# rik1599/SimplexOnCuda

Measured on AMD Instinct MI355X. Metric: simplex pivots/sec + HBM GB/s on gaussian update, dense m×n tableau, higher is better.
Workload: dtype f64

## Files before the change

simplexoncuda_amd/csrc/sx_kernels.hip:

```cpp

#include <float.h>

#include "sx_argmin.hpp"
#include "sx_common.hpp"

namespace {

__global__ __launch_bounds__(512) void k_argmin_pass1(const double *__restrict__ v, int L, TilePart *out,
                                                      const DevState *st) {
    if (st != nullptr && st->status != SX_NOT_ENDED) return;
    __shared__ double s_v[16];
    __shared__ int s_i[16];
    double mv = DBL_MAX;
    int mi = -1;
    for (int i = blockIdx.x * SX_TILE + threadIdx.x; i < L; i += SX_TILE * gridDim.x) {
        const double c = v[i];
        if (cmp_eps(c, mv) < 0) {
            mv = c;
            mi = i;
        }
    }
    block_argmin512(mv, mi, s_v, s_i);
    if (threadIdx.x == 0) {
        out[blockIdx.x].v = mv;
// ... 437 lines not shown
    double v = DBL_MAX;
    int i = -1;
    if ((int)threadIdx.x < B1) {
        double cv;
        int ci, ce;
        load_tile_sc1(enter_parts + threadIdx.x, cv, ci, ce);
        if (cmp_eps(cv, v) < 0) {
            v = cv;
            i = ci;
        }
    }
    half_argmin(v, i);
    __syncthreads();
    if (lane == 0) {
        s_v[h] = v;
        s_i[h] = i;
    }
    __syncthreads();
    if (threadIdx.x < 32) {
        v = (threadIdx.x < 8) ? s_v[threadIdx.x] : DBL_MAX;
        i = (threadIdx.x < 8) ? s_i[threadIdx.x] : -1;
        half_argmin(v, i);
        if (threadIdx.x == 0) {
            st->e_next = i;
            st->dmin_next = v;
            st->ticket_d = 0;
        }
    }
}

typedef unsigned long long u64;

__device__ __forceinline__ void drain() { asm volatile("s_waitcnt vmcnt(0)" ::: "memory"); }

#define SX_PAYBITS 11
#define SX_PAYMASK ((1u << SX_PAYBITS) - 1u)
#define SX_NOIDX 0x3FFu
__device__ __forceinline__ unsigned make_tag(unsigned B, int q) {
    return ((B & 0x7FFFu) << (6 + SX_PAYBITS)) | ((unsigned)q << SX_PAYBITS);
}

__device__ __forceinline__ void put_g(u64 *g, unsigned data, unsigned tag) {
    __hip_atomic_store(g, ((u64)tag << 32) | data, __ATOMIC_RELAXED, __HIP_MEMORY_SCOPE_AGENT);
}
__device__ __forceinline__ double gd(unsigned lo, unsigned hi) {
    return __longlong_as_double((long long)(((u64)hi << 32) | lo));
}
__device__ __forceinline__ u64 ld_sc1(const u64 *p) {
    return __hip_atomic_load(const_cast<u64 *>(p), __ATOMIC_RELAXED, __HIP_MEMORY_SCOPE_AGENT);
}
__device__ __forceinline__ unsigned ld_sc1(const unsigned *p) {
    return __hip_atomic_load(const_cast<unsigned *>(p), __ATOMIC_RELAXED, __HIP_MEMORY_SCOPE_AGENT);
}

#define SX_GB4 4
#define SX_GBS 16
#define SX_OBJ_TILES 160

__device__ __forceinline__ void st_sc1(double *p, double v) {
    __hip_atomic_store(reinterpret_cast<u64 *>(p), (u64)__double_as_longlong(v), __ATOMIC_RELAXED,
                       __HIP_MEMORY_SCOPE_AGENT);
}
__device__ __forceinline__ double ld_sc1d(const double *p) {
    return __longlong_as_double((long long)ld_sc1(reinterpret_cast<const u64 *>(p)));
}
struct IdOff {
    __device__ __forceinline__ int operator()(int k) const { return k; }
};
struct Rec4Val {
    __device__ __forceinline__ int operator()(int k) const { return (k >> 1) * SX_GBS + (k & 1); }
};
struct Rec4AllFrom {
    int k0;
    __device__ __forceinline__ int operator()(int k) const { return ((k0 + k) >> 2) * SX_GBS + ((k0 + k) & 3); }
};
struct Rec4All {
    __device__ __forceinline__ int operator()(int k) const { return (k >> 2) * SX_GBS + (k & 3); }
};

__device__ __forceinline__ u64 ld_sys(const u64 *p) {
    return __hip_atomic_load(const_cast<u64 *>(p), __ATOMIC_RELAXED, __HIP_MEMORY_SCOPE_SYSTEM);
}

#define SX_GATHER_PER_LANE 8

__device__ __forceinline__ void poll_pause() { __builtin_amdgcn_s_sleep(1); }

template <typename OFF, bool SYS, int PL, typename PAYF>
__device__ __forceinline__ int poll_wave_f(const u64 *base, int n, OFF off, unsigned tag, unsigned *out, unsigned *abort_w,
                           unsigned long long timeout, PAYF payf) {
    const int t = threadIdx.x & 63;
    const u64 t0 = __builtin_amdgcn_s_memrealtime();
    if (n <= 64) {
        bool have = t >= n;
        for (unsigned it = 0;; ++it) {
            if (!have) {
                const u64 w = SYS ? ld_sys(base + off(t)) : ld_sc1(base + off(t));
                if (((unsigned)(w >> 32) | SX_PAYMASK) == (tag | SX_PAYMASK)) {
                    have = true;
                    out[t] = (unsigned)w;
                    payf(t, (unsigned)(w >> 32) & SX_PAYMASK);
                }
            }
            if (__ballot(!have) == 0ull) return 1;
            if ((it & 63) == 63) {
                int stop = ld_sc1(abort_w) != 0u;
                if (!stop && __builtin_amdgcn_s_memrealtime() - t0 > timeout) {
                    __hip_atomic_store(abort_w, 1u, __ATOMIC_RELAXED, __HIP_MEMORY_SCOPE_AGENT);
                    stop = 1;
                }
                if (__builtin_amdgcn_readfirstlane(stop)) return 0;
            }
            poll_pause();
        }
    }
    unsigned miss = 0u;
#pragma unroll
    for (int c = 0; c < PL; ++c)
        if (t + 64 * c < n) miss |= 1u << c;
    for (unsigned it = 0;; ++it) {
        u64 w[PL];
#pragma unroll
        for (int c = 0; c < PL; ++c)
            if ((miss >> c) & 1u) w[c] = SYS ? ld_sys(base + off(t + 64 * c)) : ld_sc1(base + off(t + 64 * c));
#pragma unroll
        for (int c = 0; c < PL; ++c) {
            const int k = t + 64 * c;
            if (((miss >> c) & 1u) && ((unsigned)(w[c] >> 32) | SX_PAYMASK) == (tag | SX_PAYMASK)) {
                miss &= ~(1u << c);
                out[k] = (unsigned)w[c];
                payf(k, (unsigned)(w[c] >> 32) & SX_PAYMASK);
            }
        }
        if (__ballot(miss != 0u) == 0ull) return 1;
        if ((it & 63) == 63) {
            int stop = ld_sc1(abort_w) != 0u;
            if (!stop && __builtin_amdgcn_s_memrealtime() - t0 > timeout) {
                __hip_atomic_store(abort_w, 1u, __ATOMIC_RELAXED, __HIP_MEMORY_SCOPE_AGENT);
                stop = 1;
            }
            if (__builtin_amdgcn_readfirstlane(stop)) return 0;
        }
        poll_pause();
    }
}

template <typename OFF, bool SYS = false>
__device__ int poll_wave(const u64 *base, int n, OFF off, unsigned tag, unsigned *out, unsigned *abort_w,
                         unsigned long long timeout, unsigned *pay) {
    return poll_wave_f<OFF, SYS, SX_GATHER_PER_LANE>(base, n, off, tag, out, abort_w, timeout,
                                                     [pay](int k, unsigned pl) {
                                                         if (pay && !(k & 1)) pay[k >> 1] = pl;
                                                     });
}

template <typename OFF>
struct OffFrom {
    OFF off;
    int k0;
    __device__ __forceinline__ int operator()(int k) const { return off(k0 + k); }
};
template <typename OFF, typename PAYF>
__device__ __forceinline__ int poll_block(const u64 *base, int n, int rec, OFF off, unsigned tag, unsigned *out,
                                          unsigned *abort_w, unsigned long long timeout, PAYF payf, int *s_okw) {
    const int w = (int)threadIdx.x >> 6, nw = (int)blockDim.x >> 6;
    const int per = ((n + nw - 1) / nw + rec - 1) / rec * rec;
    const int k0 = w * per, nk = n - k0 < per ? (n - k0 > 0 ? n - k0 : 0) : per;
    int ok = 1;
    if (nk > 0)
        ok = poll_wave_f<OffFrom<OFF>, false, 2>(base, nk, OffFrom<OFF>{off, k0}, tag, out + k0, abort_w, timeout,
                                                 [&](int kl, unsigned pl) { payf(k0 + kl, pl); });
    if ((threadIdx.x & 63) == 0) s_okw[w] = ok;
    __syncthreads();
    int all = 1;
    for (int w1 = 0; w1 < nw; ++w1) all &= s_okw[w1];
    return all;
}

template <int S = 2, typename PT = unsigned>
__device__ __forceinline__ void wave_pass2(const unsigned *s_g, const PT *s_pay, int nt, double *s_v,
                                           int *s_i, double &v_out, int &i_out, int &any_elig) {
    const int lane = threadIdx.x;
    const int R = (nt + 63) >> 6;
    unsigned te = 0u;
    for (int r = 0; r < R; ++r) {
        const int p = r * 64 + lane;
        double v = DBL_MAX;
        int i = -1;
        if (p < nt) {
            const double cv = gd(s_g[S * p], s_g[S * p + 1]);
            const unsigned pl = s_pay[p];
            te |= (pl >> 10) & 1u;
            if (cmp_eps(cv, v) < 0) {
                v = cv;
                i = (pl & SX_NOIDX) == SX_NOIDX ? -1 : p * SX_TILE + (int)(pl & SX_NOIDX);
            }
        }
        half_argmin(v, i);
        if ((lane & 31) == 0) {
            s_v[2 * r + (lane >> 5)] = v;
            s_i[2 * r + (lane >> 5)] = i;
        }
    }
    double v = DBL_MAX;
    int i = -1;
    if (lane < 2 * R) {
        v = s_v[lane];
        i = s_i[lane];
    }
    half_argmin(v, i);
    any_elig = __ballot(te != 0u) != 0ull;
    v_out = v;
    i_out = i;
}

template <typename OFF, bool SYS = false>
__device__ bool gather_tagged(const u64 *base, int n, OFF off, unsigned tag, unsigned *out, unsigned *abort_w,
                              int *s_ok, unsigned long long timeout = 20000000ull, unsigned *pay = nullptr) {
    const int t = threadIdx.x, nt = blockDim.x;
    if (n <= 64 * SX_GATHER_PER_LANE) {
        if (t < 64) {
            const int ok = poll_wave<OFF, SYS>(base, n, off, tag, out, abort_w, timeout, pay);
            if (t == 0) *s_ok = ok;
        }
        __syncthreads();
        return *s_ok != 0;
    }
    unsigned have = 0u;
#pragma unroll
    for (int c = 0; c < 4; ++c)
        if (t + c * nt >= n) have |= 1u << c;
    const u64 t0 = __builtin_amdgcn_s_memrealtime();
    for (unsigned it = 0;; ++it) {
#pragma unroll
        for (int c = 0; c < 4; ++c) {
            if (!((have >> c) & 1u)) {
                const int k = t + c * nt;
                const u64 w = SYS ? ld_sys(base + off(k)) : ld_sc1(base + off(k));
                if (((unsigned)(w >> 32) | SX_PAYMASK) == (tag | SX_PAYMASK)) {
                    have |= 1u << c;
                    out[k] = (unsigned)w;
                    if (pay && !(k & 1)) pay[k >> 1] = (unsigned)(w >> 32) & SX_PAYMASK;
                }
            }
        }
        if (!__syncthreads_or(have != 0xFu)) break;
        if ((it & 63) == 63) {
            if (t == 0) {
                int stop = ld_sc1(abort_w) != 0u;
                if (!stop && __builtin_amdgcn_s_memrealtime() - t0 > timeout) {
                    __hip_atomic_store(abort_w, 1u, __ATOMIC_RELAXED, __HIP_MEMORY_SCOPE_AGENT);
                    stop = 1;
                }
                *s_ok = !stop;
            }
            __syncthreads();
            if (!*s_ok) return false;
        }
        poll_pause();
    }
    return true;
}

#define SX_GA_STRIDE (10 + 2 * SX_HMAX)
#define SX_GB_STRIDE (9 + 2 * SX_HMAX)
__device__ __forceinline__ int rec2_a(int k) { return (k >> 1) * SX_GA_STRIDE + (k & 1); }
__host__ __device__ __forceinline__ size_t sx_ga_size() { return (size_t)SX_TILE * SX_GA_STRIDE; }
__host__ __device__ __forceinline__ size_t sx_gb_size() { return (size_t)SX_TILE * SX_GB_STRIDE; }
__device__ __forceinline__ int rec2_b(int k) { return (k >> 1) * SX_GB_STRIDE + (k & 1); }

__device__ __forceinline__ double rdlane(double v, int l) {
    const long long b = __double_as_longlong(v);
    const int lo = __builtin_amdgcn_readlane((int)b, l), hi = __builtin_amdgcn_readlane((int)(b >> 32), l);
    return __longlong_as_double((long long)(((unsigned long long)(unsigned)hi << 32) | (unsigned)lo));
}


__device__ __forceinline__ double shfl_d(double v, int src) {
    const long long b = __double_as_longlong(v);
    const int lo = __shfl((int)b, src), hi = __shfl((int)(b >> 32), src);
    return __longlong_as_double((long long)(((unsigned long long)(unsigned)hi << 32) | (unsigned)lo));
}

template <int K>
__device__ __forceinline__ double fma_bc(double w, double h, double x) {
    asm("v_fmac_f64_dpp %0, %1, %2 row_newbcast:%3 row_mask:0xf bank_mask:0xf" : "+v"(x) : "v"(w), "v"(h), "n"(K));
    return x;
}
struct Bc2 {
    double w[2];
};
__device__ __forceinline__ void bc2_fence(Bc2 &b) { asm volatile("s_nop 1" : "+v"(b.w[0]), "+v"(b.w[1])); }
__device__ __forceinline__ Bc2 bc2_from_lanes(double wv) {
    const int l = (int)threadIdx.x & 15;
    Bc2 b{{shfl_d(wv, l), shfl_d(wv, 16 + l)}};
    bc2_fence(b);
    return b;
}
__device__ __forceinline__ Bc2 bc2_from_lds(const double *s_v) {
    const int l = (int)threadIdx.x & 15;
    Bc2 b{{s_v[l], s_v[16 + l]}};
    bc2_fence(b);
    return b;
}
template <int S0>
__device__ __forceinline__ double bc_steps8(double x, const Bc2 &W, const double (&h)[8], int from, int q) {
#define SX_BCS(K)                                                                       \
    if (S0 + K >= from && S0 + K < q) x = fma_bc<(S0 + K) & 15>(W.w[(S0 + K) >> 4], h[K], x);
    SX_BCS(0) SX_BCS(1) SX_BCS(2) SX_BCS(3) SX_BCS(4) SX_BCS(5) SX_BCS(6) SX_BCS(7)
#undef SX_BCS
    return x;
}
template <int S0>
__device__ __forceinline__ double bc_steps8_after(double x, const Bc2 &W, const double (&h)[8], int q, int sl,
                                                  bool all) {
#define SX_BCS(K)                                                                          \
    if (S0 + K < q) {                                                                      \
        const double y = fma_bc<(S0 + K) & 15>(W.w[(S0 + K) >> 4], h[K], x);               \
        x = (all || S0 + K > sl) ? y : x;                                                  \
    }
    SX_BCS(0) SX_BCS(1) SX_BCS(2) SX_BCS(3) SX_BCS(4) SX_BCS(5) SX_BCS(6) SX_BCS(7)
#undef SX_BCS
    return x;
}
__device__ __forceinline__ double bc_chain_lds(double x, const Bc2 &W, const double *s_hist, int from, int q) {
    const int t = threadIdx.x;
    double h[8];
#define SX_BCG(S0)                                                                     \
    if (S0 < q && S0 + 8 > from) {                                                     \
        _Pragma("unroll") for (int k = 0; k < 8; ++k) h[k] = s_hist[(S0 + k) * SX_TILE + t]; \
        x = bc_steps8<S0>(x, W, h, from, q);                                           \
    }
    SX_BCG(0) SX_BCG(8) SX_BCG(16) SX_BCG(24)
#undef SX_BCG
    return x;
}
__device__ __forceinline__ double bc_chain_lds_after(double x, const Bc2 &W, const double *s_hist, int q, int sl,
                                                     bool all) {
    const int t = threadIdx.x;
    double h[8];
#define SX_BCG(S0)                                                                     \
    if (S0 < q) {                                                                      \
        _Pragma("unroll") for (int k = 0; k < 8; ++k) h[k] = s_hist[(S0 + k) * SX_TILE + t]; \
        x = bc_steps8_after<S0>(x, W, h, q, sl, all);                                  \
    }
    SX_BCG(0) SX_BCG(8) SX_BCG(16) SX_BCG(24)
#undef SX_BCG
    return x;
}
__device__ __forceinline__ double bc_chain_regs(double x, const Bc2 &W, const double (&h1)[SX_HMAX], int from) {
    double h[8];
#define SX_BCG(S0)                                                                     \
    _Pragma("unroll") for (int k = 0; k < 8; ++k) h[k] = h1[S0 + k];                   \
    x = bc_steps8<S0>(x, W, h, from, SX_HMAX);
    SX_BCG(0) SX_BCG(8) SX_BCG(16) SX_BCG(24)
#undef SX_BCG
    return x;
}
__device__ __forceinline__ double bc_chain_regs_after(double x, const Bc2 &W, const double (&h1)[SX_HMAX], int sl,
                                                      bool all) {
    double h[8];
#define SX_BCG(S0)                                                                     \
    _Pragma("unroll") for (int k = 0; k < 8; ++k) h[k] = h1[S0 + k];                   \
    x = bc_steps8_after<S0>(x, W, h, SX_HMAX, sl, all);
    SX_BCG(0) SX_BCG(8) SX_BCG(16) SX_BCG(24)
#undef SX_BCG
    return x;
}

__device__ __forceinline__ double hist_col_bc(double a, int q, unsigned bits, const double *s_hist, double wu,
                                              const double *s_p) {
    const Bc2 W = bc2_from_lanes(wu);
    if (__ballot(bits != 0u) == 0ull) return bc_chain_lds(a, W, s_hist, 0, q);
    const int sl = bits ? 31 - __builtin_clz(bits) : 0;
    const double usl = shfl_d(wu, sl);
    if (bits) a = usl / s_p[sl];
    return bc_chain_lds_after(a, W, s_hist, q, bits ? sl : -1, !bits);
}
__device__ __forceinline__ double stage1_col_bc(double a, const double (&h)[SX_HMAX], unsigned bits, double wu,
                                                const double *s_p) {
    const Bc2 W = bc2_from_lanes(wu);
    if (__ballot(bits != 0u) == 0ull) return bc_chain_regs(a, W, h, 0);
    const int sl = bits ? 31 - __builtin_clz(bits) : 0;
    const double usl = shfl_d(wu, sl);
    if (bits) a = usl / s_p[sl];
    return bc_chain_regs_after(a, W, h, bits ? sl : -1, !bits);
}
__device__ __forceinline__ double hist_col_rl(double a, int q, unsigned bits, const double *s_hist, const double *s_ue,
                                              const double *s_p) {
    const int t = threadIdx.x, lane = t & 63;
    const double wu = s_ue[lane & (SX_HMAX - 1)];
    if (__ballot(bits != 0u) == 0ull) {
        int s = 0;
        for (; s + 8 <= q; s += 8) {
            double h[8];
#pragma unroll
            for (int k = 0; k < 8; ++k) h[k] = s_hist[(s + k) * SX_TILE + t];
#pragma unroll
            for (int k = 0; k < 8; ++k) a = fma(h[k], rdlane(wu, s + k), a);
        }
        for (; s < q; ++s) a = fma(s_hist[s * SX_TILE + t], rdlane(wu, s), a);
        return a;
    }
    const int sl = bits ? 31 - __builtin_clz(bits) : -1;
    if (bits) a = s_ue[sl] / s_p[sl];
    for (int s0 = 0; s0 < q; s0 += 8) {
        double h[8];
#pragma unroll
        for (int k = 0; k < 8; ++k) h[k] = s_hist[(s0 + k < q ? s0 + k : s0) * SX_TILE + t];
#pragma unroll
        for (int k = 0; k < 8; ++k) {
            if (s0 + k < q) {
                const double y = fma(h[k], rdlane(wu, s0 + k), a);
                a = s0 + k > sl ? y : a;
            }
        }
    }
    return a;
}
__device__ __forceinline__ double stage1_col_rl(double a, const double (&h)[SX_HMAX], unsigned bits, const double *s_u,
                                                const double *s_p) {
    const int lane = threadIdx.x & 63;
    const double wu = s_u[lane & (SX_HMAX - 1)];
    if (__ballot(bits != 0u) == 0ull) {
#pragma unroll
        for (int s = 0; s < SX_HMAX; ++s) a = fma(h[s], rdlane(wu, s), a);
        return a;
    }
    const int sl = bits ? 31 - __builtin_clz(bits) : -1;
    if (bits) a = s_u[sl] / s_p[sl];
#pragma unroll
    for (int s = 0; s < SX_HMAX; ++s) {
        const double y = fma(h[s], rdlane(wu, s), a);
        a = s > sl ? y : a;
    }
    return a;
}
__device__ __forceinline__ double hist_row_rl(double u, int q, int r, const double *s_hist, const double *s_fr,
                                              const double *s_p, const int *s_r) {
    const int t = threadIdx.x, lane = t & 63;
    const double wf = s_fr[lane & (SX_HMAX - 1)];
    const unsigned long long left = __ballot(lane < q && s_r[lane < q ? lane : 0] == r);
    int s = 0;
    if (left) {
        const int sl = 63 - __builtin_clzll(left);
        u = s_hist[sl * SX_TILE + t] / s_p[sl];
        s = sl + 1;
    }
    for (; s + 8 <= q; s += 8) {
        double h[8];
#pragma unroll
        for (int k = 0; k < 8; ++k) h[k] = s_hist[(s + k) * SX_TILE + t];
#pragma unroll
        for (int k = 0; k < 8; ++k) u = fma(rdlane(wf, s + k), h[k], u);
    }
    for (; s < q; ++s) u = fma(rdlane(wf, s), s_hist[s * SX_TILE + t], u);
    return u;
}
__device__ __forceinline__ double stage1_row_rl(double u, const double (&h)[SX_HMAX], int r, const double *s_f,
                                                const double *s_p, const int *s_r) {
    const int lane = threadIdx.x & 63;
    const double wf = s_f[lane & (SX_HMAX - 1)];
    const unsigned long long left = __ballot(lane < SX_HMAX && s_r[lane < SX_HMAX ? lane : 0] == r);
    if (left == 0ull) {
#pragma unroll
        for (int s = 0; s < SX_HMAX; ++s) u = fma(rdlane(wf, s), h[s], u);
        return u;
    }
    const int sl = 63 - __builtin_clzll(left);
    double hs = 0.0;
#pragma unroll
    for (int s = 0; s < SX_HMAX; ++s) hs = s == sl ? h[s] : hs;
    u = hs / s_p[sl];
#pragma unroll
    for (int s = 0; s < SX_HMAX; ++s) {
        const double y = fma(rdlane(wf, s), h[s], u);
        u = s > sl ? y : u;
    }
    return u;
}
__device__ __forceinline__ double hist_row_bc(double u, int q, int r, const double *s_hist, const double *s_fr,
                                              const double *s_p, const int *s_r) {
    const int t = threadIdx.x, lane = t & 63;
    const Bc2 W = bc2_from_lds(s_fr);
    const unsigned long long left = __ballot(lane < q && s_r[lane < q ? lane : 0] == r);
    int from = 0;
    if (left) {
        const int sl = 63 - __builtin_clzll(left);
        u = s_hist[sl * SX_TILE + t] / s_p[sl];
        from = sl + 1;
    }
    return bc_chain_lds(u, W, s_hist, from, q);
}
__device__ __forceinline__ double stage1_row_bc(double u, const double (&h)[SX_HMAX], int r, const double *s_f,
                                                const double *s_p, const int *s_r) {
    const int lane = threadIdx.x & 63;
    const Bc2 W = bc2_from_lds(s_f);
    const unsigned long long left = __ballot(lane < SX_HMAX && s_r[lane < SX_HMAX ? lane : 0] == r);
    if (left == 0ull) return bc_chain_regs(u, W, h, 0);
    const int sl = 63 - __builtin_clzll(left);
    double hs = 0.0;
#pragma unroll
    for (int s1 = 0; s1 < SX_HMAX; ++s1) hs = s1 == sl ? h[s1] : hs;
    u = hs / s_p[sl];
    return bc_chain_regs(u, W, h, sl + 1);
}

__device__ void activate_block(int *__restrict__ perm, int *__restrict__ iperm, int *__restrict__ ucol,
                               const int *__restrict__ urow,
                               int *__restrict__ nact_p, int m, double *__restrict__ T, int rows, TLay tl, int s0,
                               double *__restrict__ U, size_t ld, int nU, const int *s_rr, int cnt, int *s_pl,
                               int *s_ol, int *s_cl, int *s_src, int *s_misc, double *s_u) {
    const int t = threadIdx.x;
    if (t < 64) {
        const int na0 = *nact_p;
        int kc = -1, pr = 0, win = -1;
        if (t < cnt) {
            kc = ucol[s_rr[t]];
            pr = kc >= 0 ? perm[kc] : 0;
            if (na0 + t < m) win = iperm[na0 + t];
        }
        int pl = -1, ol = -1, cl = -1;
        int nl = 0, added = 0;
        for (int s = 0; s < cnt; ++s) {
            const int rs = __shfl(kc, s);
            if (rs < 0) continue;
            if (__ballot(t < nl && cl == rs && pl >= na0 && pl < na0 + added)) continue;
            const unsigned long long hP = __ballot(t < nl && cl == rs);
            int iP;
            if (hP) {
                iP = __ffsll((long long)hP) - 1;
            } else {
                iP = nl++;
                const int P = __shfl(pr, s);
                if (t == iP) {
                    pl = P;
                    ol = rs;
                    cl = rs;
                }
            }
            const int pos = na0 + added;
            const unsigned long long hW = __ballot(t < nl && pl == pos);
            int iW;
            if (hW) {
                iW = __ffsll((long long)hW) - 1;
            } else {
                iW = nl++;
                const int w = __shfl(win, added);
                if (t == iW) {
                    pl = pos;
                    ol = w;
                    cl = w;
                }
            }
            const int cP = __shfl(cl, iP), cW = __shfl(cl, iW);
            if (t == iP) cl = cW;
            if (t == iW) cl = cP;
            ++added;
        }
        if (t < nl) {
            s_pl[t] = pl;
            s_ol[t] = ol;
            s_cl[t] = cl;
        }
        if (t == 0) {
            s_misc[0] = nl;
            s_misc[1] = added;
            s_misc[2] = na0;
        }
    }
    __syncthreads();
    const int nl = s_misc[0];
    if (nl == 0) return;
    if (t < nl) {
        int j = 0;
        while (s_ol[j] != s_cl[t]) ++j;
        s_src[t] = j;
    }
    __syncthreads();
    for (int k = t; k < nU * nl; k += blockDim.x) {
        const int s = k / nl, i = k - s * nl;
        s_u[k] = __longlong_as_double(
            (long long)ld_sc1(reinterpret_cast<const u64 *>(U + (size_t)s * ld + s0 + s_pl[s_src[i]])));
    }
    __syncthreads();
    for (int k = t; k < nU * nl; k += blockDim.x) {
        const int s = k / nl, i = k - s * nl;
        U[(size_t)s * ld + s0 + s_pl[i]] = s_u[k];
    }
    if (t < nl) {
        const int x = s_pl[t], o = s_ol[t], cc = s_cl[t];
        if (o != cc) {
            const int ro = urow[o], rc = urow[cc];
            if (ro < rows) T[tl.idx(ro, s0 + x)] = 0.0;
            if (rc < rows) T[tl.idx(rc, s0 + x)] = 1.0;
        }
        iperm[x] = cc;
        perm[cc] = x;
        const int na0 = s_misc[2];
        if (x >= na0 && x < na0 + s_misc[1]) ucol[urow[cc]] = -1;
    }
    if (t == 0) *nact_p = s_misc[2] + s_misc[1];
}

[[maybe_unused]] constexpr int kRV = 0;
constexpr int kRD = 2;
constexpr int kRA = 4;
constexpr int kRB = 6;
constexpr int kRE = 8;
constexpr int kRS = 9;
constexpr int kRF = 10;
[[maybe_unused]] constexpr int kOV = 0;
constexpr int kOP = 2;
constexpr int kOB = 4;
constexpr int kOR = 6;
constexpr int kOS = 7;
constexpr int kOM = 8;
constexpr int kOU = 9;

__global__ __launch_bounds__(512) void k_batch(const double *T, int rows, size_t ld, TLay tl, Cols c,
                                               double *__restrict__ d, double *__restrict__ d_save, int *base,
                                               DevState *st, double *U, double *F, PivRec *recs,
                                               unsigned long long *PM, unsigned long long *PM2, unsigned B, int K,
                                               int NA, int NB,
                                               BatchChan *ch, u64 *ga, u64 *gb, unsigned long long *stamps,
                                               int *perm, int *iperm, int *ucol, const int *urow, int *nact, int m) {
    extern __shared__ double s_hist[];
    __shared__ double s_v[16];
    __shared__ int s_i[16];
    __shared__ double s_p[SX_KMAX];
    __shared__ int s_r[SX_KMAX], s_e[SX_KMAX];
    __shared__ double s_fr[SX_HMAX], s_fr1[SX_HMAX];
    __shared__ double s_a[SX_TILE], s_b[SX_TILE];
    __shared__ unsigned s_g[4 * SX_TILE];
    __shared__ unsigned s_pay[SX_TILE];
    __shared__ unsigned short s_payo[3 * SX_OBJ_TILES];
    __shared__ double s_uq;
    __shared__ int s_last;
    __shared__ int s_sel_ok, s_sel_r, s_sel_any, s_det_ok, s_det_e, s_det_st, s_ent_ok, s_ent_e, s_ent_m;
    __shared__ double s_det_dmin, s_ent_v, s_br, s_ent_p;
    __shared__ int s_welig[SX_TILE / 64];
    __shared__ int s_okw[SX_TILE / 64];
    const int t = threadIdx.x;
    const bool isA = (int)blockIdx.x < NA;
#define SX_STAMP(k)                                                                           \
    do {                                                                                       \
        if (stamps && t == 0) stamps[(size_t)q * 8 + (k)] = __builtin_amdgcn_s_memrealtime(); \
    } while (0)
#define SX_BSTAMP(k)                                                                                    \
    do {                                                                                                \
        if (stamps && t == 0)                                                                           \
            stamps[(size_t)K * 8 + ((size_t)q * (NA + NB) + blockIdx.x) * 4 + (k)] =                    \
                __builtin_amdgcn_s_memrealtime();                                                       \
    } while (0)
    const int status0 = st->status;
    const long long piv0 = st->pivots, cap = st->max_pivots;
    int e = st->e_next;
    double dmin = st->dmin_next;
    int status = SX_NOT_ENDED, cnt = 0;
    bool aborted = false;
    const unsigned inj = ch->inject_q;
    if (status0 == SX_NOT_ENDED) {
        const int li = blockIdx.x * SX_TILE + t;
        const bool liveA = isA && li < rows;
        const int tb = blockIdx.x - NA;
        const int L = c.N - 1;
        const int ia = tb * SX_TILE + t;
        const bool liveB = !isA && ia < L;
        const int mj = c.map(1 + (liveB ? ia : 0));
        if (!isA) reinterpret_cast<int *>(s_a)[t] = mj;
        double b = liveA ? T[tl.idx(li, 0)] : 0.0;
        unsigned bits = 0u;
        unsigned bits1 = 0u;
        double h1[SX_HMAX];
#pragma unroll
        for (int s1 = 0; s1 < SX_HMAX; ++s1) h1[s1] = 0.0;
        int hb = 0;
        double dj = liveB ? d[1 + ia] : 0.0;
        double d0 = (!isA && tb == 0 && t == 0) ? d[0] : 0.0;
        if (liveB) d_save[1 + ia] = dj;
        if (!isA && tb == 0 && t == 0) d_save[0] = d0;
        double a_pre = liveA ? T[tl.idx(li, c.map(1 + (e >= 0 ? e : 0)))] : 0.0;
        auto next_stage = [&]() {
#pragma unroll
            for (int s1 = 0; s1 < SX_HMAX; ++s1) h1[s1] = s_hist[s1 * SX_TILE + t];
            bits1 = bits;
            bits = 0u;
            drain();
            __syncthreads();
            if (t == 0) __builtin_amdgcn_fence(__ATOMIC_RELEASE, "agent");
            __syncthreads();
            hb = SX_HMAX;
        };
        if (isA) {
            double wu = 0.0, wu1 = 0.0;
            for (int q = 0; q < K; ++q) {
                const unsigned tag = make_tag(B, q);
                if (cap >= 0 && piv0 + q >= cap) {
                    status = SX_PIVOT_CAP;
                    break;
                }
                if (q == SX_HMAX) next_stage();
                if (inj != 0u && blockIdx.x == 0 && (unsigned)q + 1u == inj) {
                    if (t == 0) __hip_atomic_store(&ch->abort_w, 1u, __ATOMIC_RELAXED, __HIP_MEMORY_SCOPE_AGENT);
                    aborted = true;
                    break;
                }
                const int qq = q - hb;
                const bool done = !(cmp_eps(dmin, 0.0) < 0);
                if (blockIdx.x == 0) SX_STAMP(0);
                SX_BSTAMP(0);
                double a1 = a_pre;
                if (hb && !done) a1 = stage1_col_bc(a1, h1, bits1, wu1, s_p);
                const double a = done ? 0.0 : hist_col_bc(a1, qq, bits, s_hist, wu, s_p + hb);
                double rv = DBL_MAX;
                int ri = -1, elig = 0;
                if (liveA && !done) {
                    elig = a >= SX_EPS;
                    const double ratio = cmp_eps(a, 0.0) > 0 ? b / a : DBL_MAX;
                    if (cmp_eps(ratio, rv) < 0) {
                        rv = ratio;
                        ri = li;
                    }
                }
                if (blockIdx.x == 0) SX_STAMP(2);
                s_a[t] = a;
                s_b[t] = b;
                drain();
                half_argmin(rv, ri);
                const int anyw = __ballot(elig) != 0ull;
                if ((t & 31) == 0) {
                    s_v[t >> 5] = rv;
                    s_i[t >> 5] = ri;
                }
                if ((t & 63) == 0) s_welig[t >> 6] = anyw;
                __syncthreads();
                if (t < 64) {
                    double v = t < 16 ? s_v[t] : DBL_MAX;
                    int i = t < 16 ? s_i[t] : -1;
                    half_argmin(v, i);
                    int any = 0;
#pragma unroll
                    for (int w = 0; w < SX_TILE / 64; ++w) any |= s_welig[w];
                    const int wi = __builtin_amdgcn_readfirstlane(i);
                    const long long vb = __double_as_longlong(v);
                    const double wv = __longlong_as_double(
                        ((long long)__builtin_amdgcn_readfirstlane((int)(vb >> 32)) << 32) |
                        (long long)(unsigned)__builtin_amdgcn_readfirstlane((int)vb));
                    const int wl = wi >= 0 ? wi - (int)blockIdx.x * SX_TILE : 0;
                    const unsigned pl = (wi >= 0 ? (unsigned)wl : SX_NOIDX) | ((unsigned)any << 10);
                    const int nG = kRF + 2 * qq;
                    for (int k = t; k < nG; k += 64) {
                        unsigned data;
                        if (k == kRE) {
                            data = (unsigned)e;
                        } else if (k == kRS) {
                            data = (unsigned)(done ? SX_FEASIBLE : SX_NOT_ENDED);
                        } else {
                            const double val = k < kRD ? wv : k < kRA ? dmin : k < kRB ? s_a[wl] : k < kRE ? s_b[wl]
                                                                           : s_hist[((k - kRF) >> 1) * SX_TILE + wl];
                            const u64 bits64 = (u64)__double_as_longlong(val);
                            data = (k & 1) ? (unsigned)(bits64 >> 32) : (unsigned)bits64;
                        }
                        put_g(ga + (size_t)blockIdx.x * SX_GA_STRIDE + k, data, k < kRD ? (tag | pl) : tag);
                    }
                }
                if (blockIdx.x == 0) SX_STAMP(1);
                SX_BSTAMP(1);
                if (done) {
                    status = SX_FEASIBLE;
                    break;
                }
                if (t < 64) {
                    int ok = poll_wave(ga, 2 * NA, rec2_a, tag, s_g, &ch->abort_w, 20000000ull, s_pay);
                    double tv = DBL_MAX;
                    int ti = -1, any = 0;
                    if (ok) wave_pass2(s_g, s_pay, NA, s_v, s_i, tv, ti, any);
                    ti = __builtin_amdgcn_readfirstlane(ti);
                    if (ok && ti >= 0) {
                        const int wt = ti / SX_TILE;
                        ok = poll_wave(ga + (size_t)wt * SX_GA_STRIDE + kRA, 4, IdOff(), tag, s_g + 2048 - 64,
                                       &ch->abort_w, 20000000ull, (unsigned *)nullptr);
                    }
                    if (t == 0) {
                        s_sel_ok = ok;
                        s_sel_r = ti;
                        s_sel_any = any;
                        if (ok && ti >= 0) {
                            s_ent_p = gd(s_g[2048 - 64], s_g[2048 - 63]);
                            s_br = gd(s_g[2048 - 62], s_g[2048 - 61]);
                        }
                    }
                }
                __syncthreads();
                if (!s_sel_ok) {
                    aborted = true;
                    break;
                }
                if (!s_sel_any) {
                    status = SX_UNBOUNDED;
                    break;
                }
                const int r = s_sel_r;
                if (r < 0) {
                    status = SX_NUMERIC_FAIL;
                    break;
                }
                const double p = s_ent_p, br = s_br;
                if (t == 0) {
                    s_p[q] = p;
                    s_r[q] = r;
                    s_e[q] = e;
                }
                cnt = q + 1;
                const double f = -a / p;
                s_hist[qq * SX_TILE + t] = f;
                if (liveA) {
                    st_sc1(F + sx_fidx(li, q), f);
                    if (li == r) {
                        b = b / p;
                        bits |= 1u << qq;
                        (hb ? PM2 : PM)[li] = ((u64)B << 32) | bits;
                    } else {
                        b = fma(f, br, b);
                    }
                }
                if (blockIdx.x == 0 && t == 0) {
                    recs[q].r = r;
                    recs[q].e = e;
                    recs[q].p = p;
                    U[(size_t)q * ld] = br;
                }
                unsigned short *po = s_payo;
                const int okb = poll_block(gb, SX_GB4 * NB, SX_GB4, Rec4All(), tag, s_g, &ch->abort_w, 20000000ull,
                                           [po](int k, unsigned pl) {
                                               if ((k & 3) < 3) po[(k & 3) * SX_OBJ_TILES + (k >> 2)] = (unsigned short)pl;
                                           }, s_okw);
                if (t < 64) {
                    double ev = DBL_MAX;
                    int ei = -1, any = 0;
                    if (okb) wave_pass2<SX_GB4, unsigned short>(s_g, s_payo, NB, s_v, s_i, ev, ei, any);
                    if (t == 0) {
                        s_ent_ok = okb;
                        s_ent_e = ei;
                        s_ent_v = ev;
                        s_ent_m = 0;
                        s_uq = 0.0;
                        if (okb && ei >= 0) {
                            const int wt = ei / SX_TILE;
                            s_ent_m = (int)s_payo[SX_OBJ_TILES + wt] | ((int)s_payo[2 * SX_OBJ_TILES + wt] << SX_PAYBITS);
                            s_uq = gd(s_g[SX_GB4 * wt + 2], s_g[SX_GB4 * wt + 3]);
                        }
                    }
                }
                __syncthreads();
                if (blockIdx.x == 0) SX_STAMP(5);
                SX_BSTAMP(2);
                if (!s_ent_ok) {
                    aborted = true;
                    break;
                }
                e = s_ent_e;
                dmin = s_ent_v;
                {
                    const int me = s_ent_m, lane = t & 63, q1 = q + 1, hb1 = q1 >= SX_HMAX ? SX_HMAX : 0;
                    const double uq = s_uq;
                    if (liveA) a_pre = T[tl.idx(li, me)];
                    const int sa = hb1 + lane;
                    wu = lane < q1 - hb1 ? (sa == q ? uq : ld_sc1d(U + (size_t)sa * ld + me)) : 0.0;
                    if (hb1) wu1 = lane < SX_HMAX ? (lane == q ? uq : ld_sc1d(U + (size_t)lane * ld + me)) : 0.0;
                }
            }
        } else {
            for (int q = 0; q < K; ++q) {
                const unsigned tag = make_tag(B, q);
                if (cap >= 0 && piv0 + q >= cap) {
                    status = SX_PIVOT_CAP;
                    break;
                }
                if (q == SX_HMAX) next_stage();
                const int qq = q - hb;
                if (t < 64) {
                    const int ok = poll_wave(ga, 2 * NA, rec2_a, tag, s_g, &ch->abort_w, 20000000ull, s_pay);
                    double tv = DBL_MAX;
                    int ti = -1, any = 0;
                    if (ok) wave_pass2(s_g, s_pay, NA, s_v, s_i, tv, ti, any);
                    if (t == 0) {
                        s_sel_ok = ok;
                        s_sel_r = ti;
                        s_sel_any = any;
                    }
                }
                __syncthreads();
                if (tb == 0) SX_STAMP(3);
                SX_BSTAMP(0);
                if (!s_sel_ok) {
                    aborted = true;
                    break;
                }
                const int r = s_sel_r;
                double u = liveB && r >= 0 ? T[tl.idx(r, mj)] : 0.0;
                if (t < 64) {
                    const int wt = r >= 0 ? r / SX_TILE : 0;
                    u64 fr1 = 0ull;
                    if (hb && t < SX_HMAX)
                        fr1 = ld_sc1(reinterpret_cast<const u64 *>(F + sx_fidx(r >= 0 ? r : 0, t)));
                    const int ok = poll_wave(ga + (size_t)wt * SX_GA_STRIDE + kRD, (kRF - kRD) + 2 * qq,
                                             [](int k) { return k; }, tag, s_g, &ch->abort_w, 20000000ull,
                                             (unsigned *)nullptr);
                    if (hb && t < SX_HMAX) s_fr1[t] = __longlong_as_double((long long)fr1);
                    if (ok) {
                        if (t < qq) s_fr[t] = gd(s_g[kRF - kRD + 2 * t], s_g[kRF - kRD + 1 + 2 * t]);
                        if (t == 0) {
                            s_det_dmin = gd(s_g[0], s_g[1]);
                            s_p[q] = gd(s_g[kRA - kRD], s_g[kRA - kRD + 1]);
                            s_br = gd(s_g[kRB - kRD], s_g[kRB - kRD + 1]);
                            s_det_e = (int)s_g[kRE - kRD];
                            s_det_st = (int)s_g[kRS - kRD];
                            s_r[q] = r;
                            s_e[q] = (int)s_g[kRE - kRD];
                        }
                    }
                    if (t == 0) s_det_ok = ok;
                }
                __syncthreads();
                SX_BSTAMP(1);
                if (!s_det_ok) {
                    aborted = true;
                    break;
                }
                e = s_det_e;
                dmin = s_det_dmin;
                int ost = SX_NOT_ENDED;
                if (s_det_st != SX_NOT_ENDED) {
                    status = s_det_st;
                    break;
                }
                if (!s_sel_any) {
                    ost = SX_UNBOUNDED;
                } else if (r < 0) {
                    ost = SX_NUMERIC_FAIL;
                }
                const double p = s_p[q], br = s_br;
                double v = DBL_MAX;
                int i = -1;
                if (ost == SX_NOT_ENDED) {
                    cnt = q + 1;
                    if (tb == 0) SX_STAMP(6);
                    if (hb) u = stage1_row_bc(u, h1, r, s_fr1, s_p, s_r);
                    u = hist_row_bc(u, qq, r, s_hist, s_fr, s_p + hb, s_r + hb);
                    s_hist[qq * SX_TILE + t] = u;
                    if (tb == 0) SX_STAMP(7);
                    const double fd = -dmin / p;
                    if (tb == 0 && t == 0) d0 = fma(fd, br, d0);
                    if (liveB) {
                        dj = fma(fd, u, dj);
                        if (cmp_eps(dj, v) < 0) {
                            v = dj;
                            i = ia;
                        }
                    }
                }
                half_argmin(v, i);
                if ((t & 31) == 0) {
                    s_v[t >> 5] = v;
                    s_i[t >> 5] = i;
                }
                drain();
                __syncthreads();
                if (t < 64) {
                    double wv = t < 16 ? s_v[t] : DBL_MAX;
                    int wi = t < 16 ? s_i[t] : -1;
                    half_argmin(wv, wi);
                    wi = __builtin_amdgcn_readfirstlane(wi);
                    const long long vb = __double_as_longlong(wv);
                    wv = __longlong_as_double(((long long)__builtin_amdgcn_readfirstlane((int)(vb >> 32)) << 32) |
                                              (long long)(unsigned)__builtin_amdgcn_readfirstlane((int)vb));
                    const int win = wi >= 0 ? wi - tb * SX_TILE : 0;
                    if (t < SX_GB4) {
                        const int k = t;
                        const int mw = reinterpret_cast<const int *>(s_a)[win];
                        const double val = k < 2 ? wv : s_hist[qq * SX_TILE + win];
                        const u64 bits64 = (u64)__double_as_longlong(val);
                        const unsigned data = (k & 1) ? (unsigned)(bits64 >> 32) : (unsigned)bits64;
                        const unsigned pl = k == 0 ? (wi >= 0 ? (unsigned)win : SX_NOIDX)
                                          : k == 1 ? ((unsigned)mw & SX_PAYMASK)
                                          : k == 2 ? (((unsigned)mw >> SX_PAYBITS) & SX_PAYMASK) : 0u;
                        put_g(gb + (size_t)tb * SX_GBS + k, data, tag | pl);
                    }
                }
                if (ost == SX_NOT_ENDED && liveB && 1 + ia < c.Ns) st_sc1(U + (size_t)q * ld + mj, s_hist[qq * SX_TILE + t]);
                if (tb == 0) SX_STAMP(4);
                SX_BSTAMP(2);
                if (ost != SX_NOT_ENDED) {
                    status = ost;
                    break;
                }
            }
        }
        if (!isA && !aborted && (status == SX_NOT_ENDED || status == SX_PIVOT_CAP) && cnt > 0) {
            const unsigned tag = make_tag(B, cnt - 1);
            if (t < 64) {
                const int ok = poll_wave(gb, 2 * NB, Rec4Val(), tag, s_g, &ch->abort_w, 20000000ull, s_pay);
                double ev = DBL_MAX;
                int ei = -1, any = 0;
                if (ok) wave_pass2(s_g, s_pay, NB, s_v, s_i, ev, ei, any);
                if (t == 0) {
                    s_ent_ok = ok;
                    s_ent_e = ei;
                    s_ent_v = ev;
                }
            }
            __syncthreads();
            if (!s_ent_ok) aborted = true;
            e = s_ent_e;
            dmin = s_ent_v;
        }
        if (liveB) d[1 + ia] = dj;
        if (!isA && tb == 0 && t == 0) d[0] = d0;
    }
    drain();
    __syncthreads();
    if (t == 0) {
        __builtin_amdgcn_fence(__ATOMIC_RELEASE, "agent");
        const unsigned k = __hip_atomic_fetch_add(&ch->exit_cnt, 1u, __ATOMIC_RELAXED, __HIP_MEMORY_SCOPE_AGENT);
        s_last = k == (unsigned)(NA + NB) - 1;
        if (s_last) {
            __hip_atomic_store(&ch->exit_cnt, 0u, __ATOMIC_RELAXED, __HIP_MEMORY_SCOPE_AGENT);
            if (inj != 0u) ch->inject_q = 0u;
        }
    }
    __syncthreads();
    if (!s_last || status0 != SX_NOT_ENDED) return;
    const bool hang = ld_sc1(&ch->abort_w) != 0u || aborted;
    if (!hang && perm != nullptr && cnt > 0) {
        for (int s1 = 0; s1 < cnt; s1 += SX_HMAX) {
            if (s1) __syncthreads();
            activate_block(perm, iperm, ucol, urow, nact, m, const_cast<double *>(T), rows, tl, c.s0, U, ld, cnt, s_r + s1,
                           cnt - s1 < SX_HMAX ? cnt - s1 : SX_HMAX, reinterpret_cast<int *>(s_g),
                           reinterpret_cast<int *>(s_g) + 64, reinterpret_cast<int *>(s_g) + 128,
                           reinterpret_cast<int *>(s_g) + 192, reinterpret_cast<int *>(s_pay), s_hist);
        }
    }
    if (t != 0) return;
    if (hang) {
        st->status = SX_HANG;
        __hip_atomic_store(&ch->abort_w, 0u, __ATOMIC_RELAXED, __HIP_MEMORY_SCOPE_AGENT);
        return;
    }
    for (int s = 0; s < cnt; ++s) base[s_r[s]] = s_e[s];
    st->status = status;
    st->pivots = piv0 + cnt;
    if (cnt > 0) {
        st->r = s_r[cnt - 1];
        st->e = s_e[cnt - 1];
        st->batch_tag = B;
        st->batch_count = cnt;
    }
    st->e_next = e;
    st->dmin_next = dmin;
#undef SX_STAMP
#undef SX_BSTAMP
}


__device__ __forceinline__ void put_g_sys(u64 *g, unsigned data, unsigned tag) {
    __hip_atomic_store(g, ((u64)tag << 32) | data, __ATOMIC_RELAXED, __HIP_MEMORY_SCOPE_SYSTEM);
}
__device__ __forceinline__ void st_sys(double *p, double v) {
    __hip_atomic_store(reinterpret_cast<u64 *>(p), (u64)__double_as_longlong(v), __ATOMIC_RELAXED,
                       __HIP_MEMORY_SCOPE_SYSTEM);
}
__device__ __forceinline__ double ld_sys(const double *p) {
    return __longlong_as_double((long long)ld_sys(reinterpret_cast<const u64 *>(p)));
}

__device__ __forceinline__ void batch_mr_body(int bid, unsigned nbl, const double *__restrict__ T, int rows, int row0,
                                              int rpr, size_t ld, TLay tl, Cols c, double *__restrict__ d,
                                              double *__restrict__ d_save, int *base, DevState *st, double *U, double *F,
                                              PivRec *recs, unsigned long long *PM, unsigned long long *PM2, unsigned B,
                                              int K, int slots, int W,
                                              int rank, int tb0, int tb1, int NBg, int repl, BatchChan *ch,
                                              const u64 *ga, const u64 *gb, const u64 *gdone, PeerView pv,
                                              unsigned long long timeout) {
    extern __shared__ double s_hist[];
    __shared__ double s_v[16];
    __shared__ int s_i[16];
    __shared__ double s_p[SX_KMAX];
    __shared__ int s_r[SX_KMAX], s_e[SX_KMAX];
    __shared__ double s_ue[SX_KMAX], s_fr[SX_KMAX];
    __shared__ double s_ue1[SX_HMAX], s_fr1[SX_HMAX];
    __shared__ double s_a[SX_TILE], s_b[SX_TILE];
    __shared__ unsigned s_g[4 * SX_TILE];
    __shared__ unsigned s_pay[SX_TILE];
    __shared__ int s_ok, s_flag;
    __shared__ int s_sel_ok, s_sel_r, s_sel_any, s_det_ok, s_det_e, s_det_st, s_ent_ok, s_ent_e, s_ent_r, s_ent_st, s_ent_m;
    __shared__ double s_det_dmin, s_ent_v, s_br, s_ent_p;
    __shared__ int s_welig[SX_TILE / 64];
    const int t = threadIdx.x;
    const bool isA = bid < slots;
    const int NAg = W * slots;
    const int status0 = st->status;
    const long long piv0 = st->pivots, cap = st->max_pivots;
    int e = st->e_next;
    double dmin = st->dmin_next;
    int status = SX_NOT_ENDED, cnt = 0;
    bool aborted = false;
    const unsigned inj = ch->inject_q;
    auto gather_a = [](int k) { return rec2_a(k); };
    auto gather_b = [](int k) { return rec2_b(k); };
    auto ident = [](int k) { return k; };
    const int li = bid * SX_TILE + t;
    const bool liveA = isA && li < rows;
    const int gt = rank * slots + bid;
    const int tb = tb0 + bid - slots;
    const int L = c.N - 1;
    const int ia = tb * SX_TILE + t;
    const bool liveB = !isA && ia < L;
    const int mj = c.map(1 + (liveB ? ia : 0));
    if (!isA) reinterpret_cast<int *>(s_a)[t] = mj;
    double dj = liveB ? d[1 + ia] : 0.0;
    double d0 = (!isA && tb == 0 && t == 0) ? d[0] : 0.0;
// ... 1663 lines not shown
```

Baseline: 38150.

## Poll pivot-row header per wave and read eta coefficients directly from F

Each wave now polls the pivot-row header with its own lanes (poll_lanes) and broadcasts the values via readlane, instead of wave 0 polling into shared memory and then a __syncthreads. The eta factor column is loaded straight from F into lanes rather than being published through the gather array, so the producer writes only the fixed header. The left-row check uses a register ballot over past pivot rows, which skips the T load and stage-1 chain when the row was already pivoted. The goal is to remove one block barrier and the shared-memory round trip per pivot, at the cost of more redundant polling traffic and abort/status checks deferred to the later barrier.

```diff
diff --git a/simplexoncuda_amd/csrc/sx_kernels.hip b/simplexoncuda_amd/csrc/sx_kernels.hip
--- a/simplexoncuda_amd/csrc/sx_kernels.hip
+++ b/simplexoncuda_amd/csrc/sx_kernels.hip
@@ -613,6 +613,33 @@
                                                      [pay](int k, unsigned pl) {
                                                          if (pay && !(k & 1)) pay[k >> 1] = pl;
                                                      });
+}
+
+__device__ __forceinline__ int poll_lanes(const u64 *base, int n, unsigned tag, unsigned &out, unsigned *abort_w,
+                                          unsigned long long timeout) {
+    const int lane = threadIdx.x & 63;
+    const u64 t0 = __builtin_amdgcn_s_memrealtime();
+    bool have = lane >= n;
+    out = 0u;
+    for (unsigned it = 0;; ++it) {
+        if (!have) {
+            const u64 w = ld_sc1(base + lane);
+            if (((unsigned)(w >> 32) | SX_PAYMASK) == (tag | SX_PAYMASK)) {
+                have = true;
+                out = (unsigned)w;
+            }
+        }
+        if (__ballot(!have) == 0ull) return 1;
+        if ((it & 63) == 63) {
+            int stop = ld_sc1(abort_w) != 0u;
+            if (!stop && __builtin_amdgcn_s_memrealtime() - t0 > timeout) {
+                __hip_atomic_store(abort_w, 1u, __ATOMIC_RELAXED, __HIP_MEMORY_SCOPE_AGENT);
+                stop = 1;
+            }
+            if (__builtin_amdgcn_readfirstlane(stop)) return 0;
+        }
+        poll_pause();
+    }
 }
 
 template <typename OFF>
@@ -758,12 +785,6 @@
     bc2_fence(b);
     return b;
 }
-__device__ __forceinline__ Bc2 bc2_from_lds(const double *s_v) {
-    const int l = (int)threadIdx.x & 15;
-    Bc2 b{{s_v[l], s_v[16 + l]}};
-    bc2_fence(b);
-    return b;
-}
 template <int S0>
 __device__ __forceinline__ double bc_steps8(double x, const Bc2 &W, const double (&h)[8], int from, int q) {
 #define SX_BCS(K)                                                                       \
@@ -940,26 +961,23 @@
     }
     return u;
 }
-__device__ __forceinline__ double hist_row_bc(double u, int q, int r, const double *s_hist, const double *s_fr,
-                                              const double *s_p, const int *s_r) {
-    const int t = threadIdx.x, lane = t & 63;
-    const Bc2 W = bc2_from_lds(s_fr);
-    const unsigned long long left = __ballot(lane < q && s_r[lane < q ? lane : 0] == r);
+__device__ __forceinline__ double hist_row_bc(double u, int q, unsigned left, const double *s_hist, double wf,
+                                              const double *s_p) {
+    const int t = threadIdx.x;
+    const Bc2 W = bc2_from_lanes(wf);
     int from = 0;
     if (left) {
-        const int sl = 63 - __builtin_clzll(left);
+        const int sl = 31 - __builtin_clz(left);
         u = s_hist[sl * SX_TILE + t] / s_p[sl];
         from = sl + 1;
     }
     return bc_chain_lds(u, W, s_hist, from, q);
 }
-__device__ __forceinline__ double stage1_row_bc(double u, const double (&h)[SX_HMAX], int r, const double *s_f,
-                                                const double *s_p, const int *s_r) {
-    const int lane = threadIdx.x & 63;
-    const Bc2 W = bc2_from_lds(s_f);
-    const unsigned long long left = __ballot(lane < SX_HMAX && s_r[lane < SX_HMAX ? lane : 0] == r);
-    if (left == 0ull) return bc_chain_regs(u, W, h, 0);
-    const int sl = 63 - __builtin_clzll(left);
+__device__ __forceinline__ double stage1_row_bc(double u, const double (&h)[SX_HMAX], unsigned left, double wf,
+                                                const double *s_p) {
+    const Bc2 W = bc2_from_lanes(wf);
+    if (left == 0u) return bc_chain_regs(u, W, h, 0);
+    const int sl = 31 - __builtin_clz(left);
     double hs = 0.0;
 #pragma unroll
     for (int s1 = 0; s1 < SX_HMAX; ++s1) hs = s1 == sl ? h[s1] : hs;
@@ -1091,15 +1109,14 @@
     __shared__ int s_i[16];
     __shared__ double s_p[SX_KMAX];
     __shared__ int s_r[SX_KMAX], s_e[SX_KMAX];
-    __shared__ double s_fr[SX_HMAX], s_fr1[SX_HMAX];
     __shared__ double s_a[SX_TILE], s_b[SX_TILE];
     __shared__ unsigned s_g[4 * SX_TILE];
     __shared__ unsigned s_pay[SX_TILE];
     __shared__ unsigned short s_payo[3 * SX_OBJ_TILES];
     __shared__ double s_uq;
     __shared__ int s_last;
-    __shared__ int s_sel_ok, s_sel_r, s_sel_any, s_det_ok, s_det_e, s_det_st, s_ent_ok, s_ent_e, s_ent_m;
-    __shared__ double s_det_dmin, s_ent_v, s_br, s_ent_p;
+    __shared__ int s_sel_ok, s_sel_r, s_sel_any, s_ent_ok, s_ent_e, s_ent_m;
+    __shared__ double s_ent_v, s_br, s_ent_p;
     __shared__ int s_welig[SX_TILE / 64];
     __shared__ int s_okw[SX_TILE / 64];
     const int t = threadIdx.x;
@@ -1210,16 +1227,15 @@
                         (long long)(unsigned)__builtin_amdgcn_readfirstlane((int)vb));
                     const int wl = wi >= 0 ? wi - (int)blockIdx.x * SX_TILE : 0;
                     const unsigned pl = (wi >= 0 ? (unsigned)wl : SX_NOIDX) | ((unsigned)any << 10);
-                    const int nG = kRF + 2 * qq;
-                    for (int k = t; k < nG; k += 64) {
+                    if (t < kRF) {
+                        const int k = t;
                         unsigned data;
                         if (k == kRE) {
                             data = (unsigned)e;
                         } else if (k == kRS) {
                             data = (unsigned)(done ? SX_FEASIBLE : SX_NOT_ENDED);
                         } else {
-                            const double val = k < kRD ? wv : k < kRA ? dmin : k < kRB ? s_a[wl] : k < kRE ? s_b[wl]
-                                                                           : s_hist[((k - kRF) >> 1) * SX_TILE + wl];
+                            const double val = k < kRD ? wv : k < kRA ? dmin : k < kRB ? s_a[wl] : s_b[wl];
                             const u64 bits64 = (u64)__double_as_longlong(val);
                             data = (k & 1) ? (unsigned)(bits64 >> 32) : (unsigned)bits64;
                         }
@@ -1333,6 +1349,8 @@
                 }
             }
         } else {
+            const int lane = t & 63;
+            int wr = -1;
             for (int q = 0; q < K; ++q) {
                 const unsigned tag = make_tag(B, q);
                 if (cap >= 0 && piv0 + q >= cap) {
@@ -1360,56 +1378,53 @@
                     break;
                 }
                 const int r = s_sel_r;
-                double u = liveB && r >= 0 ? T[tl.idx(r, mj)] : 0.0;
-                if (t < 64) {
-                    const int wt = r >= 0 ? r / SX_TILE : 0;
-                    u64 fr1 = 0ull;
-                    if (hb && t < SX_HMAX)
-                        fr1 = ld_sc1(reinterpret_cast<const u64 *>(F + sx_fidx(r >= 0 ? r : 0, t)));
-                    const int ok = poll_wave(ga + (size_t)wt * SX_GA_STRIDE + kRD, (kRF - kRD) + 2 * qq,
-                                             [](int k) { return k; }, tag, s_g, &ch->abort_w, 20000000ull,
-                                             (unsigned *)nullptr);
-                    if (hb && t < SX_HMAX) s_fr1[t] = __longlong_as_double((long long)fr1);
-                    if (ok) {
-                        if (t < qq) s_fr[t] = gd(s_g[kRF - kRD + 2 * t], s_g[kRF - kRD + 1 + 2 * t]);
-                        if (t == 0) {
-                            s_det_dmin = gd(s_g[0], s_g[1]);
-                            s_p[q] = gd(s_g[kRA - kRD], s_g[kRA - kRD + 1]);
-                            s_br = gd(s_g[kRB - kRD], s_g[kRB - kRD + 1]);
-                            s_det_e = (int)s_g[kRE - kRD];
-                            s_det_st = (int)s_g[kRS - kRD];
-                            s_r[q] = r;
-                            s_e[q] = (int)s_g[kRE - kRD];
-                        }
-                    }
-                    if (t == 0) s_det_ok = ok;
-                }
-                __syncthreads();
-                SX_BSTAMP(1);
-                if (!s_det_ok) {
-                    aborted = true;
-                    break;
-                }
-                e = s_det_e;
-                dmin = s_det_dmin;
+                const u64 leftb = r >= 0 ? __ballot(wr == r) : 0ull;
+                const unsigned left = (unsigned)(leftb >> hb);
+                const unsigned left1 = hb ? (unsigned)leftb : 0u;
+                const int rr = r >= 0 ? r : 0;
+                double wf = 0.0, wf1 = 0.0;
+                if (lane < qq) wf = ld_sc1d(F + sx_fidx(rr, hb + lane));
+                if (hb && !left && lane < SX_HMAX) wf1 = ld_sc1d(F + sx_fidx(rr, lane));
+                double u = 0.0;
+                if (leftb == 0ull && liveB && r >= 0) u = T[tl.idx(r, mj)];
+                unsigned g;
+                const int okw = poll_lanes(ga + (size_t)(rr / SX_TILE) * SX_GA_STRIDE + kRD, kRF - kRD, tag, g,
+                                           &ch->abort_w, 20000000ull);
+                if (stamps && t == 0) {
+                    unsigned long long *sp = stamps + (size_t)K * 8 + ((size_t)q * (NA + NB) + blockIdx.x) * 4;
+                    sp[1] = __builtin_amdgcn_s_memrealtime();
+                    sp[3] = left ? 1u : left1 ? 2u : 0u;
+                }
+                const auto gl = [g](int k) { return (unsigned)__builtin_amdgcn_readlane((int)g, k); };
+                const auto gv = [g](int k) {
+                    unsigned x;
+                    asm("v_mov_b32 %0, %1" : "=v"(x) : "s"(__builtin_amdgcn_readlane((int)g, k)));
+                    return x;
+                };
+                const double p = gd(gv(kRA - kRD), gv(kRA - kRD + 1)), br = gd(gv(kRB - kRD), gv(kRB - kRD + 1));
+                const int rst = okw ? (int)gl(kRS - kRD) : SX_NOT_ENDED;
+                e = (int)gl(kRE - kRD);
+                dmin = gd(gv(0), gv(1));
+                if (lane == 0) {
+                    s_okw[t >> 6] = okw;
+                    s_p[q] = p;
+                    s_r[q] = r;
+                    s_e[q] = e;
+                }
+                wr = lane == q ? r : wr;
                 int ost = SX_NOT_ENDED;
-                if (s_det_st != SX_NOT_ENDED) {
-                    status = s_det_st;
-                    break;
-                }
                 if (!s_sel_any) {
                     ost = SX_UNBOUNDED;
                 } else if (r < 0) {
                     ost = SX_NUMERIC_FAIL;
                 }
-                const double p = s_p[q], br = s_br;
+                const bool run = rst == SX_NOT_ENDED && ost == SX_NOT_ENDED;
                 double v = DBL_MAX;
                 int i = -1;
-                if (ost == SX_NOT_ENDED) {
-                    cnt = q + 1;
+                if (run) {
                     if (tb == 0) SX_STAMP(6);
-                    if (hb) u = stage1_row_bc(u, h1, r, s_fr1, s_p, s_r);
-                    u = hist_row_bc(u, qq, r, s_hist, s_fr, s_p + hb, s_r + hb);
+                    if (hb && !left) u = stage1_row_bc(u, h1, left1, wf1, s_p);
+                    u = hist_row_bc(u, qq, left, s_hist, wf, s_p + hb);
                     s_hist[qq * SX_TILE + t] = u;
                     if (tb == 0) SX_STAMP(7);
                     const double fd = -dmin / p;
@@ -1429,6 +1444,20 @@
                 }
                 drain();
                 __syncthreads();
+                {
+                    int all = 1;
+#pragma unroll
+                    for (int w1 = 0; w1 < SX_TILE / 64; ++w1) all &= s_okw[w1];
+                    if (!all) {
+                        aborted = true;
+                        break;
+                    }
+                }
+                if (rst != SX_NOT_ENDED) {
+                    status = rst;
+                    break;
+                }
+                if (run) cnt = q + 1;
                 if (t < 64) {
                     double wv = t < 16 ? s_v[t] : DBL_MAX;
                     int wi = t < 16 ? s_i[t] : -1;
```

After: 38400, median of 6. Within noise of the previous version (+0.7%).
